# mckerrigan/shadow

Measured on AMD Instinct MI355X. Metric: source-paths/sec, higher is better.
Workload: dtype f64; 1 GPU; c4_as50k: Barabasi-Albert Internet-like topology, all-pairs latency/reliability table (BASELINE.json configs[3]); n_vertices=50000, n_edges=550000, n_edges_nonloop=500000, csr_arcs=1000000, targets=50000, table_bytes=40000000000, parallelism=one GPU

## Files before the change

### shadow_amd/csrc/sssp_delta.hpp

```cpp
#pragma once
#include "common.hpp"

namespace shd {

constexpr int KD_P = 8;
static_assert(KD_P == 8, "owner markers are read as one u64 per lane");
constexpr int KD_TAIL = 4;
constexpr int KD_W = 8;
constexpr int KD_IMP = 192;
constexpr uint32_t KD_NONE = 0xFFFFFFFFu;
constexpr uint32_t KD_SRC_MARK = 0xFFFFFFFEu;

#define KD_GLOBAL __attribute__((address_space(1)))

#ifndef KD_NSEEDS
#define KD_NSEEDS 3
#endif
constexpr int KD_SEEDS = KD_NSEEDS;
#ifndef KD_NTLOAD
#define KD_NTLOAD 1
#endif
#ifndef KD_JUMPS
#define KD_JUMPS 1
#endif
// ... 9 lines not shown
};
static_assert(sizeof(KDJob) == 64, "one 64-byte job record");
constexpr uint32_t KD_EVTAG = 0xFFFF0000u;
typedef unsigned short kd_us2 __attribute__((ext_vector_type(2)));
typedef double kd_d2 __attribute__((ext_vector_type(2)));
typedef unsigned kd_u4 __attribute__((ext_vector_type(4)));
typedef unsigned kd_u2 __attribute__((ext_vector_type(2)));

struct DevDelta {
    int* next;
    const KDJob* __restrict__ jobs;
    const uint16_t* __restrict__ drow;
    uint16_t* drow_out;
    uint32_t* prow;
    long long rstride;
    int evcap;
    int* done;
    int n, nw;
    int nlight;
    int nnz;
    int bound;
    int delta;
    int fused;
    int rc;
    const int* __restrict__ row;
    const uint32_t* __restrict__ orec;
    const uint16_t* __restrict__ oridx;
    const int* __restrict__ lrow;
    const uint2* __restrict__ lrec;
    const double* __restrict__ rtab;
    int nrtab;
    int rone;
    int walk;
    int packed;
    const double* __restrict__ vf;
    const double* __restrict__ self_w;
    const double* __restrict__ self_r;
    int has_vf;
    int dflags;
    int seed_drop;
    unsigned long long* dbg;
    unsigned long long* stats;
};

constexpr int KD_NACC = 40;
#ifdef SHD_STAMPS
#define KD_ACCP (sm->acc)
#define KD_OUT (!(dflags & 1))
#define KD_DFLAGS g.dflags
#define KD_STAMP(slot) do { if (tid == 0) sm->acc[slot] = __builtin_amdgcn_s_memtime(); } while (0)
#define KD_COUNT(slot, x) do { if (lane == 0 && (x)) atomicAdd(&sm->acc[slot], (unsigned long long)(x)); } while (0)
#define KD_MARK() do { if (tid == 0) kd_t = __builtin_amdgcn_s_memtime(); } while (0)
#define KD_ACC(slot) do { if (tid == 0) { const unsigned long long t_ = __builtin_amdgcn_s_memtime(); sm->acc[slot] += t_ - kd_t; kd_t = t_; } } while (0)
#define KD_FLUSH() do { lds_barrier(); if (g.dbg && i >= 0) for (int q_ = tid; q_ < KD_NACC; q_ += B) g.dbg[(size_t)i * KD_NACC + q_] = sm->acc[q_]; lds_barrier(); if (tid < KD_NACC) sm->acc[tid] = 0; lds_barrier(); } while (0)
#else
#define KD_ACCP nullptr
#define KD_OUT true
#define KD_DFLAGS 0
#define KD_STAMP(slot) do { } while (0)
#define KD_COUNT(slot, x) do { } while (0)
#define KD_MARK() do { } while (0)
#define KD_ACC(slot) do { } while (0)
#define KD_FLUSH() do { } while (0)
#endif

struct KDOut {
    const KD_GLOBAL int* tgt;
    KD_GLOBAL double* lat_out;
    KD_GLOBAL double* rel_out;
    KD_GLOBAL double* row_min;
    int* err;
    KD_GLOBAL double* relv;
    const KD_GLOBAL double* rtab;
    const KD_GLOBAL double* vf;
    long long ld;
    int n, nw, nt, tsorted;
    unsigned rmask;
    int rc, walk, nrtab, rone, has_vf, dflags;
};

struct KDSmall {
    unsigned gmin[2];
    int head, tail;
    int busy;
    int nexit;
    int rtail, rdone;
    int qtail[2];
    int qcur[2];
    unsigned long long rmin;
    int deep;
    int next;
    int nev;
    int evovf;
    int tsorted;
    int jflag[3];
    int wnext;
    int wnext2, novf;
    KDJob job;
    KDJob njob;
    int njb;
    int wpar;
    const KDJob* jobs;
    int* qnext;
    const uint16_t* drow;
    uint32_t* prow;
    long long rstride;
    int* done;
    uint32_t* wsl[2];
    int ns;
    KDOut out;
#ifdef SHD_STAMPS
    unsigned long long acc[KD_NACC];
#endif
};

template <int B>
struct KDLayout {
    size_t tmask, tpre, wmark, wkey, wimp, dist, pend, fix, wmin, work, ring, rrec, qv, qbeg, rix, rtabl, total;
    int qcap;
    __host__ __device__ static KDLayout make(int n, int rc, int rr) {
        KDLayout L;
        const size_t nw = (size_t)(n + 63) / 64;
        size_t o = a16(sizeof(KDSmall));
        L.tmask = o; o += a16(8 * nw);
        L.tpre = o;  o += a16(4 * nw);
        L.dist = o;  o += a16(sizeof(uint16_t) * (size_t)(n + 1));
        L.rix = o;
        L.wmark = o; o += (size_t)(B / 64) * 8 * KD_P;
        L.wkey = o;  o += (size_t)(B / 64) * 64 * 4;
        L.wimp = o;  o += (size_t)(B / 64) * KD_IMP * 4;
        L.pend = o;  o += a16(8 * nw);
        L.fix = o;   o += a16(8 * nw);
        L.wmin = o;  o += a16(4 * nw);
        L.work = o;
        const size_t wbytes = a16(2 * (size_t)rc) + 8 * (size_t)rr;
        L.ring = o;
        L.rrec = o + a16(2 * (size_t)rc);
        L.qcap = (int)((wbytes - 16) / 6) & ~7;
        L.qv = o;
        L.qbeg = o + a16(2 * (size_t)L.qcap);
        o += wbytes;
        L.total = o;
        L.rtabl = a16(L.rix + (size_t)n);
        return L;
    }
};
constexpr int KD_MAXD = 32;
#ifndef KD_SDIV
#define KD_SDIV 8
#endif
#ifndef KD_SMIN
#define KD_SMIN 16
#endif
#ifndef KD_WDYN
#define KD_WDYN 1
#endif
#ifndef KD_WCAP
#define KD_WCAP 2
#endif
#ifndef KD_SEEDSPIN
#define KD_SEEDSPIN 8
#endif
#ifndef KD_WQ_N
#define KD_WQ_N 2
#endif
constexpr int KD_WQ = KD_WQ_N;
constexpr int KD_ONE = 254;
constexpr int KD_NAN = 255;
constexpr int KD_RR = 512;
template <int B>
constexpr int kd_rr() { return B >= 1024 ? KD_RR : 256; }

__host__ __device__ inline size_t kd_ws_stride(int n) {
    return a16(sizeof(double) * n) + a16(sizeof(uint32_t) * (n + 8)) + a16(8 * (size_t)n) + 256 +
           a16(sizeof(uint32_t) * (n + 8));
}
__host__ __device__ inline size_t kd_ws_wpr1(int n) {
    return a16(sizeof(double) * n) + a16(sizeof(uint32_t) * (n + 8)) + a16(8 * (size_t)n) + 256;
}
__host__ __device__ inline long long kd_row_stride(int n) { return ((long long)n + 2 + 7) & ~7ll; }

__device__ inline void lds_barrier() { asm volatile("s_waitcnt lgkmcnt(0)\n\ts_barrier" ::: "memory"); }
__device__ inline void wait_stores() { asm volatile("s_waitcnt vmcnt(0)" ::: "memory"); }

__device__ inline unsigned kd_wave_min(unsigned x) {
#pragma unroll
    for (int d = 32; d >= 1; d >>= 1) x = min(x, (unsigned)__shfl_xor((int)x, d, 64));
    return x;
}

__device__ inline unsigned kd_wave_min_dpp(unsigned x) {
    int v = (int)x;
    const int inf = (int)0xFFFFFFFFu;
    v = (int)min((unsigned)v, (unsigned)__builtin_amdgcn_update_dpp(inf, v, 0x111, 0xF, 0xF, false));
    v = (int)min((unsigned)v, (unsigned)__builtin_amdgcn_update_dpp(inf, v, 0x112, 0xF, 0xF, false));
    v = (int)min((unsigned)v, (unsigned)__builtin_amdgcn_update_dpp(inf, v, 0x114, 0xF, 0xF, false));
    v = (int)min((unsigned)v, (unsigned)__builtin_amdgcn_update_dpp(inf, v, 0x118, 0xF, 0xF, false));
    v = (int)min((unsigned)v, (unsigned)__builtin_amdgcn_update_dpp(inf, v, 0x142, 0xA, 0xF, false));
    v = (int)min((unsigned)v, (unsigned)__builtin_amdgcn_update_dpp(inf, v, 0x143, 0xC, 0xF, false));
    return (unsigned)__builtin_amdgcn_readlane(v, 63);
}

__device__ inline int kd_wave_incl_sum(int x) {
    x += __builtin_amdgcn_update_dpp(0, x, 0x111, 0xF, 0xF, false);
    x += __builtin_amdgcn_update_dpp(0, x, 0x112, 0xF, 0xF, false);
    x += __builtin_amdgcn_update_dpp(0, x, 0x114, 0xF, 0xF, false);
    x += __builtin_amdgcn_update_dpp(0, x, 0x118, 0xF, 0xF, false);
    x += __builtin_amdgcn_update_dpp(0, x, 0x142, 0xA, 0xF, false);
    x += __builtin_amdgcn_update_dpp(0, x, 0x143, 0xC, 0xF, false);
    return x;
}

__device__ inline int kd_wave_incl_max(int x) {
    x = max(x, __builtin_amdgcn_update_dpp(0, x, 0x111, 0xF, 0xF, false));
    x = max(x, __builtin_amdgcn_update_dpp(0, x, 0x112, 0xF, 0xF, false));
// ... 57 lines not shown
        if (act) {
            uint32_t old = dist32[v >> 1];
            for (;;) {
                if (nd >= ((old >> sh) & 0xFFFFu)) break;
                const uint32_t got = atomicCAS(&dist32[v >> 1], old, (old & ~(0xFFFFu << sh)) | (nd << sh));
                if (got == old) { won = true; break; }
                old = got;
            }
        }
        const bool push = won && nd < T;
        if (won && nd >= T) { atomicOr(&pend[v >> 6], 1ull << (v & 63)); atomicMin(&wmin[v >> 6], nd); }
        const unsigned long long pm = __ballot(push);
        if (pm) {
            const int ctot = __popcll(pm);
            int qb = 0;
            if (lane == 0) qb = atomicAdd(tail, ctot);
            qb = __builtin_amdgcn_readfirstlane(qb);
            const int qk = max(0, min(ctot, rc - qb));
            const int rk = __popcll(pm & (upto >> 1));
            if (push && rk < qk) { ring[qb + rk] = (uint16_t)v; atomicAnd(&pend[v >> 6], ~(1ull << (v & 63))); }
            if (push && rk >= qk) { atomicOr(&pend[v >> 6], 1ull << (v & 63)); atomicMin(&wmin[v >> 6], nd); }
#ifdef SHD_STAMPS
            if (lane == 0 && ctot > qk) atomicAdd(&sm_acc[14], (unsigned long long)(ctot - qk));
#endif
        }
    }
    __builtin_amdgcn_wave_barrier();
}


#define SEED_VIEW()                                                                                   \
    const int nseed = __builtin_amdgcn_readfirstlane(sm->job.nseed);                                   \
    int su[KD_SEEDS], sslot[KD_SEEDS];                                                                 \
    unsigned wsu[KD_SEEDS], rsu[KD_SEEDS];                                                             \
    const uint16_t* sdrow[KD_SEEDS];                                                                   \
    const uint32_t* sprow[KD_SEEDS];                                                                   \
    _Pragma("unroll") for (int q_ = 0; q_ < KD_SEEDS; q_++) {                                          \
        const int sl_ = __builtin_amdgcn_readfirstlane(q_ < nseed ? sm->job.seed[q_] : 0);             \
        const unsigned wr_ = (unsigned)__builtin_amdgcn_readfirstlane(q_ < nseed ? sm->job.wr[q_] : 0); \
        su[q_] = __builtin_amdgcn_readfirstlane(q_ < nseed ? sm->job.u[q_] : -1);                      \
        sslot[q_] = sl_; wsu[q_] = wr_ & 0xFFFFu;                                                      \
        rsu[q_] = (unsigned)__builtin_amdgcn_readfirstlane(q_ < nseed ? sm->job.rec[q_] : 0);          \
        sdrow[q_] = g.drow + (size_t)sl_ * g.rstride;                                                  \
        sprow[q_] = g.prow + (size_t)sl_ * g.rstride;                                                  \
    }                                                                                                  \
    (void)sslot; (void)rsu; (void)sprow; (void)su

__device__ inline int kd_next_source(int* ctr, int* slot, int tid, bool all_queued = false) {
    if (tid == 0) *slot = (all_queued ? 0 : (int)gridDim.x) + atomicAdd(ctr, 1);
    __syncthreads();
    const int i = *slot;
    __syncthreads();
    return i;
}

template <int B>
__device__ __attribute__((noinline)) void kd_output(const int i, const int s, const double cs, const double sw_s,
                                                    const double sr_s, const KD_GLOBAL uint32_t* __restrict__ wpr) {
    extern __shared__ __attribute__((aligned(16))) char smem[];
    constexpr int RR = kd_rr<B>();
    KDSmall* sm = reinterpret_cast<KDSmall*>(smem);
    auto uni = [](auto x) __attribute__((always_inline)) {
        using T = decltype(x);
        if constexpr (sizeof(T) == 8) {
            unsigned long long b;
            __builtin_memcpy(&b, &x, 8);
            b = (unsigned long long)(unsigned)__builtin_amdgcn_readfirstlane((int)(unsigned)b) |
                ((unsigned long long)(unsigned)__builtin_amdgcn_readfirstlane((int)(unsigned)(b >> 32)) << 32);
            T y;
            __builtin_memcpy(&y, &b, 8);
            return y;
        } else {
            return (T)__builtin_amdgcn_readfirstlane((int)x);
        }
    };
    const KDOut& O = sm->out;
    const KD_GLOBAL int* __restrict__ const tgt = uni(O.tgt);
    KD_GLOBAL double* __restrict__ const lat_out = uni(O.lat_out);
    KD_GLOBAL double* __restrict__ const rel_out = uni(O.rel_out);
    KD_GLOBAL double* __restrict__ const row_min = uni(O.row_min);
    int* __restrict__ const err = uni(O.err);
    KD_GLOBAL double* __restrict__ const relv = uni(O.relv);
    const KD_GLOBAL double* __restrict__ const rtab = uni(O.rtab);
    const KD_GLOBAL double* __restrict__ const vf = uni(O.vf);
    const long long ld = uni(O.ld);
    const int n = uni(O.n), nw = uni(O.nw), nt = uni(O.nt), tsorted = uni(O.tsorted);
    const unsigned rmask = uni(O.rmask);
    const int rc = uni(O.rc), walk = uni(O.walk), nrtab = uni(O.nrtab), rone = uni(O.rone);
    const int has_vf = uni(O.has_vf), dflags = uni(O.dflags);
    const KDLayout<B> L = KDLayout<B>::make(n, rc, RR);
    const int tid = threadIdx.x, lane = tid & 63;
    uint16_t* dist = reinterpret_cast<uint16_t*>(smem + L.dist);
    unsigned long long* pend = reinterpret_cast<unsigned long long*>(smem + L.pend);
    unsigned long long* fix = reinterpret_cast<unsigned long long*>(smem + L.fix);
    uint16_t* qv = reinterpret_cast<uint16_t*>(smem + L.qv);
    const unsigned long long* tmask = reinterpret_cast<const unsigned long long*>(smem + L.tmask);
    const unsigned* tpre = reinterpret_cast<const unsigned*>(smem + L.tpre);
    const int qcap = L.qcap;
    auto tpos = [&](int v) __attribute__((always_inline)) {
        const unsigned long long wd = tmask[v >> 6], bit = 1ull << (v & 63);
        return (wd & bit) ? (int)tpre[v >> 6] + __popcll(wd & (bit - 1ull)) : -1;
    };
    struct { int walk; const KD_GLOBAL double* rtab; int nrtab; const KD_GLOBAL double* vf; int has_vf; } g = {walk, rtab, nrtab, vf, has_vf};
#ifdef SHD_STAMPS
    unsigned long long kd_t = __builtin_amdgcn_s_memtime();
#endif
    (void)lane; (void)dflags;
    KD_GLOBAL double* lrow = lat_out && i >= 0 ? lat_out + (long long)i * ld : nullptr;
    KD_GLOBAL double* rrow = rel_out && i >= 0 ? rel_out + (long long)i * ld : nullptr;
    double lmin = INFINITY;
    auto lat_of = [&](int t) __attribute__((always_inline)) {
        double Lv;
        if (t < 0 || t >= n) { raise_err(err, SHD_ROUTE_EINVAL); Lv = NAN; }
        else if (t == s) {
            if (isnan(sw_s)) { raise_err(err, SHD_ROUTE_ENOEDGE); Lv = NAN; }
            else { Lv = 0.0 + sw_s; lmin = fmin(lmin, Lv); }
        } else if (dist[t] == 0xFFFFu) { raise_err(err, SHD_ROUTE_EUNREACH); Lv = NAN; }
        else { Lv = (double)dist[t]; lmin = fmin(lmin, Lv); }
        return Lv;
    };
    const bool walks = g.walk && rrow;
    wait_stores();
    __syncthreads();
    if (tsorted) {
        const int lpar = (int)(((uintptr_t)lrow >> 3) & 1);
        const int wv = tid >> 6;
        for (int b0 = 256 * wv; b0 < (i >= 0 ? n : 0); b0 += 256 * (B / 64)) {
#pragma unroll
            for (int p = 0; p < 2; p++) {
                const int v = b0 + 128 * p + 2 * lane;
                if (v >= n) continue;
                const unsigned long long wd = tmask[v >> 6];
                const int sh = v & 63;
                const int j = (int)tpre[v >> 6] + __popcll(wd & ((1ull << sh) - 1ull));
                const uint32_t d2 = *reinterpret_cast<const uint32_t*>(dist + v);
                int jq[2];
                double Lq[2];
                int jn = j;
#pragma unroll
                for (int h = 0; h < 2; h++) {
                    const int vv = v + h;
                    const bool tg = vv < n && ((wd >> (sh + h)) & 1ull);
                    jq[h] = tg ? jn++ : -1;
                    const unsigned d = (d2 >> (16 * h)) & 0xFFFFu;
                    double Lv = 0.0;
                    if (tg) {
                        if (vv == s) {
                            if (isnan(sw_s)) { raise_err(err, SHD_ROUTE_ENOEDGE); Lv = NAN; }
                            else { Lv = 0.0 + sw_s; lmin = fmin(lmin, Lv); }
                        } else if (d == 0xFFFFu) { raise_err(err, SHD_ROUTE_EUNREACH); Lv = NAN; }
                        else { Lv = (double)d; lmin = fmin(lmin, Lv); }
                    }
                    Lq[h] = Lv;
                }
                if (!lrow || !KD_OUT) continue;
                const int ja = jq[0], jb = jq[1];
                if (ja >= 0 && jb == ja + 1 && !((ja + lpar) & 1))
                    __builtin_nontemporal_store(kd_d2{Lq[0], Lq[1]}, reinterpret_cast<KD_GLOBAL kd_d2*>(lrow + ja));
                else {
                    if (ja >= 0) __builtin_nontemporal_store(Lq[0], lrow + ja);
                    if (jb >= 0) __builtin_nontemporal_store(Lq[1], lrow + jb);
                }
            }
        }
    } else {
        for (int j = tid; j < (i >= 0 ? nt : 0); j += B) {
            const double Lv = lat_of(tgt[j]);
            if (lrow && KD_OUT) __builtin_nontemporal_store(Lv, lrow + j);
        }
    }
    const bool queued = sm->jobs != nullptr;
    if (tid == 0) {
        sm->deep = 0; sm->rmin = kInfBits; sm->wnext = 0; sm->wnext2 = 0; sm->novf = 0;
        if (queued) sm->njb = atomicAdd(sm->qnext, 1);
    }
    __syncthreads();
    const int njb = queued ? __builtin_amdgcn_readfirstlane(sm->njb) : -1;
    if (tid < 16 && njb >= 0) {
        const int x = njb < sm->ns ? ((const KD_GLOBAL int*)(sm->jobs + njb))[tid] : (tid == 3 ? 0 : -1);
        reinterpret_cast<int*>(&sm->njob)[tid] = x;
    }

    KD_ACC(18);
    uint16_t* parv = dist;
    if (walks) {
        uint8_t* rixl = reinterpret_cast<uint8_t*>(smem + L.rix);
        double* rtl = reinterpret_cast<double*>(smem + L.rtabl);
        for (int k = tid; k < 256; k += B)
            rtl[k] = k < g.nrtab ? g.rtab[k] : k == KD_ONE ? 1.0 : NAN;
        auto copy_trip = [&](const int v0, const auto& pr) __attribute__((always_inline)) {
            constexpr int NQ = sizeof(pr) / sizeof(pr[0]);
            uint2 dv[NQ];
#pragma unroll
            for (int q = 0; q < NQ; q++) dv[q] = *reinterpret_cast<const uint2*>(dist + min(v0 + q * 4 * B, (n - 1) & ~3));
#pragma unroll
            for (int q = 0; q < NQ; q++) {
                const int vb = v0 + q * 4 * B;
                if (vb >= n) continue;
                uint32_t pw[2] = {0u, 0u}, rw = 0u;
#pragma unroll
                for (int h = 0; h < 4; h++) {
                    const int v = vb + h;
                    const uint32_t p = h == 0 ? pr[q].x : h == 1 ? pr[q].y : h == 2 ? pr[q].z : pr[q].w;
                    const uint32_t d = ((h < 2 ? dv[q].x : dv[q].y) >> (16 * (h & 1))) & 0xFFFFu;
                    const bool src_v = v == s, unr = !src_v && d == 0xFFFFu;
                    const uint32_t pv = src_v || unr ? (uint32_t)s : (p & 0xFFFFu);
                    const uint32_t ri = min((p >> 16) & rmask, (uint32_t)(g.nrtab - 1));
                    const uint32_t rx = src_v ? (uint32_t)KD_ONE : unr ? (uint32_t)KD_NAN
                                        : ri == (uint32_t)rone ? (uint32_t)KD_ONE : ri;
                    pw[h >> 1] |= pv << (16 * (h & 1));
                    rw |= rx << (8 * h);
                }
                if (vb + 4 <= n) {
                    *reinterpret_cast<uint2*>(parv + vb) = make_uint2(pw[0], pw[1]);
                    *reinterpret_cast<uint32_t*>(rixl + vb) = rw;
                } else {
                    for (int h = 0; h < n - vb; h++) {
                        parv[vb + h] = (uint16_t)((pw[h >> 1] >> (16 * (h & 1))) & 0xFFFFu);
                        rixl[vb + h] = (uint8_t)((rw >> (8 * h)) & 0xFFu);
                    }
                }
            }
        };
        auto load_trip = [&](const int v0, auto& pr) __attribute__((always_inline)) {
            constexpr int NQ = sizeof(pr) / sizeof(pr[0]);
#pragma unroll
// ... 307 lines not shown
            double xp[4], xv[4];
#pragma unroll
            for (int q = 0; q < 4; q++) {
                xp[q] = relv[p4[q]];
                xv[q] = relv[v4[q] >= 0 ? v4[q] : 0];
            }
#pragma unroll
            for (int q = 0; q < 4; q++)
                if (v4[q] >= 0) relv[v4[q]] = xp[q] * (-xv[q]);
        }
        wait_stores();
        KD_ACC(14);
        lds_barrier();
        for (int k = tid; k < nw; k += B) {
            const unsigned long long r = fix[k];
            if (r) pend[k] &= ~r;
        }
        lds_barrier();
        KD_ACC(15);
    }
    KD_STAMP(3);

    if (rrow) {
        for (int j0 = tid; j0 < nt; j0 += B * 4) {
            int t4[4];
            double x4[4], f4[4];
#pragma unroll
            for (int q = 0; q < 4; q++) {
                const int j = j0 + q * B;
                t4[q] = j < nt ? tgt[j] : s;
            }
#pragma unroll
            for (int q = 0; q < 4; q++) {
                const int t = (t4[q] >= 0 && t4[q] < n) ? t4[q] : s;
                x4[q] = relv[t];
                f4[q] = g.has_vf ? g.vf[t] : (double)NAN;
            }
#pragma unroll
            for (int q = 0; q < 4; q++) {
                const int j = j0 + q * B;
                if (j >= nt) continue;
                const int t = t4[q];
                double Rv = NAN;
                if (t >= 0 && t < n) {
                    if (t == s) Rv = isnan(sw_s) ? NAN : cs * sr_s;
                    else Rv = isnan(f4[q]) ? x4[q] : x4[q] * f4[q];
                }
                if (KD_OUT) __builtin_nontemporal_store(Rv, rrow + j);
            }
        }
    }
    }
    if (row_min && i >= 0) {
#pragma unroll
        for (int d = 32; d >= 1; d >>= 1) lmin = fmin(lmin, __shfl_xor(lmin, d, 64));
        if (lane == 0 && lmin < INFINITY) atomicMin(&sm->rmin, as_u(lmin));
        __syncthreads();
        if (tid == 0) row_min[i] = as_d(sm->rmin);
    }
}

#define KD_KERNEL_PARAMS                                                                                   \
    DevDelta g, const int* __restrict__ src, int ns, const int* __restrict__ tgt, int nt, long long ld,     \
        double* __restrict__ lat_out, double* __restrict__ rel_out, double* __restrict__ row_min,          \
        int* __restrict__ err, char* __restrict__ ws, size_t ws_stride
template <int B>
__device__ __attribute__((always_inline)) inline void kd_rows_body(KD_KERNEL_PARAMS) {
    extern __shared__ __attribute__((aligned(16))) char smem[];
    const int n = g.n, nw = g.nw;
    constexpr int RR = kd_rr<B>();
    const KDLayout<B> L = KDLayout<B>::make(n, g.rc, RR);
    KDSmall* sm = reinterpret_cast<KDSmall*>(smem);
    const int tid = threadIdx.x, lane = tid & 63, wid = tid >> 6;
    uint32_t* wkey = reinterpret_cast<uint32_t*>(smem + L.wkey) + wid * 64;
    uint32_t* wimp = reinterpret_cast<uint32_t*>(smem + L.wimp) + wid * KD_IMP;
    uint16_t* dist = reinterpret_cast<uint16_t*>(smem + L.dist);
    uint32_t* wmark = reinterpret_cast<uint32_t*>(smem + L.wmark) + wid * 2 * KD_P;
    unsigned long long* pend = reinterpret_cast<unsigned long long*>(smem + L.pend);
    unsigned* wmin = reinterpret_cast<unsigned*>(smem + L.wmin);
    unsigned long long* fix = reinterpret_cast<unsigned long long*>(smem + L.fix);
    uint16_t* ring = reinterpret_cast<uint16_t*>(smem + L.ring);
    uint2* rrec = reinterpret_cast<uint2*>(smem + L.rrec);
    uint16_t* qv = reinterpret_cast<uint16_t*>(smem + L.qv);
    int* qbeg = reinterpret_cast<int*>(smem + L.qbeg);
    unsigned long long* tmask = reinterpret_cast<unsigned long long*>(smem + L.tmask);
    unsigned* tpre = reinterpret_cast<unsigned*>(smem + L.tpre);
    const unsigned delta = (unsigned)g.delta;
    const int qcap = L.qcap;
    const unsigned wmask = g.packed ? 0xFFu : 0xFFFFu;
    const unsigned rmask = g.packed ? 0xFFu : 0xFFFFu;
    const __amdgpu_buffer_rsrc_t orsrc =
        __builtin_amdgcn_make_buffer_rsrc(const_cast<uint32_t*>(g.orec), (short)0, g.nnz * 4, 0x00020000);
    const int rc = g.rc;
    constexpr int NW = B / 64;
    const bool writer = wid == NW - 1;
    double* relv = reinterpret_cast<double*>(ws + (size_t)blockIdx.x * ws_stride);
    uint32_t* const wslice = reinterpret_cast<uint32_t*>(ws + (size_t)blockIdx.x * ws_stride + a16(sizeof(double) * n));
    uint2* const evl = reinterpret_cast<uint2*>(ws + (size_t)blockIdx.x * ws_stride + a16(sizeof(double) * n) +
                                                a16(sizeof(uint32_t) * (n + 8)));
#ifdef SHD_STAMPS
    if (tid < KD_NACC) sm->acc[tid] = 0;
    __syncthreads();
#endif
    const unsigned long long upto = lane == 63 ? ~0ull : ((2ull << lane) - 1ull);

    for (int k = tid; k < nw; k += B) tmask[k] = 0ull;
    if (tid == 0) sm->tsorted = 1;
    __syncthreads();
    for (int j = tid; j < nt; j += B) {
        const int t = tgt[j];
        const bool ok = t >= 0 && t < n && (j == 0 || tgt[j - 1] < t);
        if (!ok) sm->tsorted = 0;
        else atomicOr(&tmask[t >> 6], 1ull << (t & 63));
    }
    __syncthreads();
    if (wid == 0) {
        int run = 0;
        for (int k0 = 0; k0 < nw; k0 += 64) {
            const int k = k0 + lane;
            const int c = k < nw ? __popcll(tmask[k]) : 0;
            const int incl = kd_wave_incl_sum(c);
            if (k < nw) tpre[k] = (unsigned)(run + incl - c);
            run += __builtin_amdgcn_readlane(incl, 63);
        }
    }
    __syncthreads();
    const bool tsorted = __builtin_amdgcn_readfirstlane(sm->tsorted) != 0;

    const bool queued = g.jobs != nullptr;
    if (tid == 0) {
        sm->njb = -1; sm->wpar = 0;
        sm->jobs = g.jobs; sm->qnext = g.next; sm->drow = g.drow; sm->prow = g.prow; sm->rstride = g.rstride;
        sm->done = g.done; sm->ns = ns;
        sm->wsl[0] = wslice;
        sm->wsl[1] = reinterpret_cast<uint32_t*>(ws + (size_t)blockIdx.x * ws_stride + kd_ws_wpr1(n));
        KDOut& o = sm->out;
        o.tgt = (const KD_GLOBAL int*)tgt; o.lat_out = (KD_GLOBAL double*)lat_out; o.rel_out = (KD_GLOBAL double*)rel_out;
        o.row_min = (KD_GLOBAL double*)row_min; o.err = err; o.relv = (KD_GLOBAL double*)relv;
        o.rtab = (const KD_GLOBAL double*)g.rtab; o.vf = (const KD_GLOBAL double*)g.vf; o.ld = ld;
        o.n = n; o.nw = nw; o.nt = nt; o.tsorted = tsorted ? 1 : 0; o.rmask = rmask; o.rc = g.rc; o.walk = g.walk;
        o.nrtab = g.nrtab; o.rone = g.rone; o.has_vf = g.has_vf; o.dflags = KD_DFLAGS;
    }
    for (int jb = queued ? kd_next_source(g.next, &sm->next, tid, true) : (int)blockIdx.x; jb < ns;
         jb = sm->njb >= 0 ? sm->njb : kd_next_source(g.next, &sm->next, tid, queued)) {
        if (tid < 16) {
            int x;
            if (sm->njb >= 0) x = reinterpret_cast<const int*>(&sm->njob)[tid];
            else if (g.jobs) x = reinterpret_cast<const int*>(g.jobs + jb)[tid];
            else x = tid == 0 ? jb : tid == 1 ? src[jb] : tid == 2 ? -1 : 0;
            reinterpret_cast<int*>(&sm->job)[tid] = x;
        }
        if (tid == 0) sm->wpar ^= 1;
        __syncthreads();
        if (tid == 0) sm->njb = -1;
        const int i = sm->job.row, s = sm->job.s;
        {
            bool bad = s < 0 || s >= n || sm->job.nseed < 0 || sm->job.nseed > KD_SEEDS;
            for (int q = 0; q < KD_SEEDS; q++)
                if (q < sm->job.nseed) bad = bad || sm->job.u[q] < 0 || sm->job.u[q] >= n || sm->job.seed[q] < 0;
            if (bad) {
                if (tid == 0) raise_err(err, SHD_ROUTE_EINVAL);
                __syncthreads();
                continue;
            }
        }
        auto wpr_of = [&]() __attribute__((always_inline)) {
            const int st = __builtin_amdgcn_readfirstlane(sm->job.store);
            return st >= 0 ? g.prow + (size_t)st * g.rstride : sm->wsl[__builtin_amdgcn_readfirstlane(sm->wpar)];
        };
        const double fs = g.vf[s];
        const double cs = isnan(fs) ? 1.0 : 1.0 * fs;
        const double sw_s = g.self_w[s], sr_s = g.self_r[s];
    kd_restart:
#ifdef SHD_STAMPS
        unsigned long long kd_t = 0;
#endif
        KD_MARK();
#ifdef SHD_STAMPS
        wait_stores();
        KD_ACC(9);
#endif
        const bool seeded = __builtin_amdgcn_readfirstlane(sm->job.nseed) > 0;
        if (seeded) {
            uint32_t* const wpr = wpr_of();
            if (tid == 0) {
#ifdef SHD_STAMPS
// ... 39 lines not shown
                for (int q = 0; q < KD_SEEDS; q++) {
                    if (q < nseed) {
                        if constexpr (B >= 1024 && KD_NTLOAD) {
                            typedef unsigned u2v __attribute__((ext_vector_type(2)));
                            const u2v d2 = __builtin_nontemporal_load(reinterpret_cast<const u2v*>(sdrow[q] + vl));
                            const kd_u4 p4 = __builtin_nontemporal_load(reinterpret_cast<const kd_u4*>(sprow[q] + vl));
                            dq[q] = make_uint2(d2.x, d2.y);
                            pq[q] = make_uint4(p4.x, p4.y, p4.z, p4.w);
                        } else {
                            dq[q] = *reinterpret_cast<const uint2*>(sdrow[q] + vl);
                            pq[q] = *reinterpret_cast<const uint4*>(sprow[q] + vl);
                        }
                    } else {
                        dq[q] = make_uint2(0xFFFFFFFFu, 0xFFFFFFFFu);
                        pq[q] = make_uint4(KD_NONE, KD_NONE, KD_NONE, KD_NONE);
                    }
                }
                uint32_t dw[2], rw[4];
#pragma unroll
                for (int h = 0; h < 4; h++) {
                    const int v = v0 + h;
                    unsigned dbest = 0xFFFFu, kbest = 0xFFFFFFFFu;
                    uint32_t rbest = KD_NONE;
#pragma unroll
                    for (int q = 0; q < KD_SEEDS; q++) {
                        const uint32_t d2 = (h < 2) ? dq[q].x : dq[q].y;
                        const unsigned d = (h & 1) ? (d2 >> 16) : (d2 & 0xFFFFu);
                        const unsigned c = q < nseed ? min(0xFFFFu, wsu[q] + d) : 0xFFFFFu;
                        const uint32_t p = kd_comp(pq[q], h);
                        const uint32_t r = v == su[q] ? rsu[q] : p;
                        const uint32_t k = __builtin_amdgcn_perm(~r, r, 0x07010002u);
                        if (c < dbest || (c == dbest && k < kbest)) { dbest = c; kbest = k; rbest = r; }
                    }
                    if (v >= n) dbest = 0xFFFFu;
                    if (v == s) rbest = KD_SRC_MARK;
                    if (h & 1) dw[h >> 1] |= dbest << 16;
                    else dw[h >> 1] = dbest;
                    rw[h] = rbest;
                }
                *reinterpret_cast<uint2*>(dist + v0) = make_uint2(dw[0], dw[1]);
                *reinterpret_cast<uint4*>(wpr + v0) = make_uint4(rw[0], rw[1], rw[2], rw[3]);
            }
            wait_stores();
        } else {
            for (int v = tid; v < (n + 2) / 2; v += B) reinterpret_cast<uint32_t*>(dist)[v] = 0xFFFFFFFFu;
        }
        for (int k = tid; k < nw; k += B) { pend[k] = 0ull; wmin[k] = 0xFFFFFFFFu; fix[k] = 0ull; }
        for (int q = tid; q < RR; q += B) rrec[q] = make_uint2(0u, 0xFFFFFFFFu);
        if (lane < 2 * KD_P) wmark[lane] = 0u;
        if (tid == 0) {
            sm->gmin[0] = sm->gmin[1] = 0xFFFFFFFFu;
            sm->rtail = sm->rdone = 0;
            sm->nev = 0; sm->evovf = 0;
            wpr_of()[s] = KD_SRC_MARK;
        }
        lds_barrier();
        KD_ACC(29);
        KD_STAMP(0);
        if (tid == 0) {
            dist[s] = 0;
            pend[s >> 6] = 1ull << (s & 63);
            wmin[s >> 6] = 0;
        }
        lds_barrier();

        unsigned T = delta;
        int par = 0;
        const int ncomp = NW - 1;
        int wnev = 0;
        KD_MARK();
        for (;;) {
            KD_COUNT(5, tid == 0 ? 1 : 0);
            {
                unsigned m0 = 0xFFFFFFFFu;
                for (int k = tid; k < nw; k += B) m0 = min(m0, wmin[k]);
                const unsigned wm = kd_wave_min_dpp(m0);
                if (lane == 0 && wm != 0xFFFFFFFFu) atomicMin(&sm->gmin[par], wm);
            }
            for (int q = tid; q < rc; q += B) ring[q] = 0xFFFFu;
            if (tid == 0) { sm->gmin[par ^ 1] = 0xFFFFFFFFu; sm->head = sm->tail = 0; sm->busy = 0; sm->nexit = 0; }
            lds_barrier();
            const unsigned m = sm->gmin[par];
            if (m == 0xFFFFFFFFu) break;
            if (m >= T) T = (m / delta + 1) * delta;
            KD_ACC(11);
            for (int k0 = 0; k0 < nw; k0 += B) {
                const int k = k0 + tid;
                unsigned long long bits = 0ull, take = 0ull;
                unsigned rest = 0xFFFFFFFFu;
                const bool act = k < nw && wmin[k] < T;
                if (act) {
                    bits = pend[k];
                    unsigned long long b = bits;
                    while (b) {
                        int v4[4];
                        pop4(&b, k, v4);
                        unsigned d4[4];
#pragma unroll
                        for (int q = 0; q < 4; q++) d4[q] = ld16(dist, v4[q] >= 0 ? v4[q] : n);
#pragma unroll
                        for (int q = 0; q < 4; q++) {
                            if (v4[q] < 0) continue;
                            if (d4[q] < T) take |= 1ull << (v4[q] & 63);
                            else rest = min(rest, d4[q]);
                        }
                    }
// ... 333 lines not shown
            SEED_VIEW();
            auto d0 = [&](int v) __attribute__((always_inline)) {
                unsigned x = 0xFFFFu;
#pragma unroll
                for (int q = 0; q < KD_SEEDS; q++)
                    if (q < nseed) x = min(x, min(0xFFFFu, wsu[q] + (unsigned)sdrow[q][v]));
                return x;
            };
            KD_ACC(27);
            uint32_t* key = reinterpret_cast<uint32_t*>(relv);
            auto event = [&](int e, int& v, uint32_t& ke) __attribute__((always_inline)) {
                const uint2 r = evl[e];
                v = (int)r.y;
                const int p = (int)(r.x & 0xFFFFu);
                const unsigned w = r.x >> 24, dv = ld16(dist, v);
                if (dv != d0(v) || ld16(dist, p) + w != dv) { v = -1; return; }
                ke = ((0xFFu - w) << 24) | ((uint32_t)p << 8) | ((r.x >> 16) & 0xFFu);
            };
            for (int e = tid; e < nev; e += B) {
                int v; uint32_t ke = 0;
                event(e, v, ke);
                if (v >= 0) {
                    const uint32_t b = wpr[v];
                    const unsigned pb = b & 0xFFFFu, wb = ld16(dist, v) - ld16(dist, (int)pb);
                    key[v] = ((0xFFu - wb) << 24) | (pb << 8) | ((b >> 16) & 0xFFu);
                }
            }
            wait_stores();
            lds_barrier();
            for (int e = tid; e < nev; e += B) {
                int v; uint32_t ke = 0;
                event(e, v, ke);
                if (v >= 0) atomicMin(&key[v], ke);
            }
            wait_stores();
            lds_barrier();
            for (int e = tid; e < nev; e += B) {
                int v; uint32_t ke = 0;
                event(e, v, ke);
                if (v >= 0) {
                    const uint32_t k = __hip_atomic_load(&key[v], __ATOMIC_RELAXED, __HIP_MEMORY_SCOPE_AGENT);
                    wpr[v] = ((k >> 8) & 0xFFFFu) | ((k & 0xFFu) << 16) | ((0xFFu - (k >> 24)) << 24);
                }
            }
            wait_stores();
            lds_barrier();
            KD_ACC(28);
        }
        KD_STAMP(1);
        KD_MARK();

        const int last_arc = g.nlight > 0 ? g.nlight - 1 : 0;
        uint32_t* const wpr = wpr_of();
        if (tid == 0) {
            fix[s >> 6] &= ~(1ull << (s & 63));
            sm->qtail[0] = sm->qtail[1] = 0;
            sm->qcur[0] = sm->qcur[1] = 0;
        }
        for (int rnd = 0;; rnd ^= 1) {
            if (tid == 0) { sm->qtail[rnd ^ 1] = 0; sm->qcur[rnd ^ 1] = 0; }
            lds_barrier();
            for (int k0 = 0; k0 < nw; k0 += B) {
                const int k = k0 + tid;
                unsigned long long bits = k < nw ? fix[k] : 0ull;
                const int cnt = __popcll(bits);
                int incl = kd_wave_incl_sum(cnt);
                int base = 0;
                if (lane == 63 && incl) base = atomicAdd(&sm->qtail[rnd], incl);
                base = __builtin_amdgcn_readlane(base, 63);
                int pos = base + incl - cnt;
                unsigned long long b = bits, listed = 0ull;
                while (b && pos < qcap) {
                    const int bi = __ffsll((long long)b) - 1;
                    b &= b - 1;
                    qv[pos++] = (uint16_t)((k << 6) + bi);
                    listed |= 1ull << bi;
                }
                if (listed) fix[k] = bits & ~listed;
            }
            lds_barrier();
            const int cnt = min(sm->qtail[rnd], qcap);
            if (cnt == 0) break;
            for (int j0 = 0; j0 < cnt; j0 += B * 4) {
                int v4[4], a4[4], r4[4];
#pragma unroll
                for (int q = 0; q < 4; q++) {
                    const int j = j0 + q * B + tid;
                    v4[q] = j < cnt ? (int)qv[j] : -1;
                }
#pragma unroll
                for (int q = 0; q < 4; q++) {
                    const int vv = v4[q] >= 0 ? v4[q] : 0;
                    a4[q] = g.lrow[vv];
                    r4[q] = g.lrow[vv + 1];
                }
                uint2 rc[4][KD_TAIL];
#pragma unroll
                for (int q = 0; q < 4; q++)
#pragma unroll
                    for (int e = 0; e < KD_TAIL; e++) rc[q][e] = g.lrec[min(a4[q] + e, last_arc)];
                unsigned dt[4][KD_TAIL], d4[4];
#pragma unroll
                for (int q = 0; q < 4; q++) {
                    d4[q] = ld16(dist, v4[q] >= 0 ? v4[q] : 0);
#pragma unroll
                    for (int e = 0; e < KD_TAIL; e++) dt[q][e] = ld16(dist, (int)(rc[q][e].x & 0xFFFFu));
// ... 8 lines not shown
                        if (a4[q] + e < r4[q] && dt[q][e] + (rc[q][e].x >> 16) == d4[q]) {
                            f = e;
                            rec = (rc[q][e].x & 0xFFFFu) | (rc[q][e].y << 16) | (g.packed ? (rc[q][e].x >> 16) << 24 : 0u);
                        }
                    out_a[q] = rec;
                    if (v4[q] >= 0 && f < 0) {
                        if (r4[q] - a4[q] > KD_TAIL) {
                            const int at = atomicAdd(&sm->qcur[rnd], 1);
                            qbeg[at] = v4[q];
                            v4[q] = -1;
                        } else raise_err(err, SHD_ROUTE_EUNREACH);
                    }
                }
#pragma unroll
                for (int q = 0; q < 4; q++)
                    if (v4[q] >= 0) wpr[v4[q]] = out_a[q];
            }
            lds_barrier();
            const int nlong = sm->qcur[rnd];
            for (int j = wid; j < nlong; j += B / 64) {
                const int v = qbeg[j];
                const unsigned dv = ld16(dist, v);
                const int r1 = g.lrow[v + 1];
                uint32_t fr = KD_NONE;
                for (int a0 = g.lrow[v] + KD_TAIL; a0 < r1 && fr == KD_NONE; a0 += 64) {
                    const int a = a0 + lane;
                    const uint2 rc = g.lrec[min(a, last_arc)];
                    const bool tight = a < r1 && ld16(dist, (int)(rc.x & 0xFFFFu)) + (rc.x >> 16) == dv;
                    const unsigned long long tm = __ballot(tight);
                    if (tm) fr = (uint32_t)__builtin_amdgcn_readlane((int)((rc.x & 0xFFFFu) | (rc.y << 16) | (g.packed ? (rc.x >> 16) << 24 : 0u)),
                                                                  __ffsll((long long)tm) - 1);
                }
                if (lane == 0) {
                    if (fr == KD_NONE) raise_err(err, SHD_ROUTE_EUNREACH);
                    wpr[v] = fr;
                }
            }
        }
        KD_ACC(16);
        KD_ACC(17);
        const int store = __builtin_amdgcn_readfirstlane(sm->job.store);
        if (store >= 0) {
            uint16_t* dr = g.drow_out + (size_t)store * g.rstride;
            for (int v0 = 8 * tid; v0 <= n; v0 += 8 * B)
                *reinterpret_cast<uint4*>(dr + v0) = *reinterpret_cast<const uint4*>(dist + v0);
            wait_stores();
            __syncthreads();
            if (tid == 0) {
                __builtin_amdgcn_fence(__ATOMIC_RELEASE, "agent");
                asm volatile("s_waitcnt vmcnt(0)" ::: "memory");
                __hip_atomic_store(&g.done[store], 1, __ATOMIC_RELAXED, __HIP_MEMORY_SCOPE_AGENT);
            }
        }
        KD_STAMP(2);
        kd_output<B>(i, s, cs, sw_s, sr_s, (const KD_GLOBAL uint32_t*)wpr);
        lds_barrier();
        KD_STAMP(4);
        KD_FLUSH();
    }
}

template <int B>
__global__ __launch_bounds__(B) __attribute__((amdgpu_waves_per_eu(4))) void sssp_delta_kernel(KD_KERNEL_PARAMS) {
    kd_rows_body<B>(g, src, ns, tgt, nt, ld, lat_out, rel_out, row_min, err, ws, ws_stride);
}
template <int B>
__global__ __launch_bounds__(B) __attribute__((amdgpu_waves_per_eu(4))) void kd_plan_rows_kernel(KD_KERNEL_PARAMS) {
    kd_rows_body<B>(g, src, ns, tgt, nt, ld, lat_out, rel_out, row_min, err, ws, ws_stride);
}

template <int B>
inline size_t kd_lds_bytes(int n, int rc) { return KDLayout<B>::make(n, rc, kd_rr<B>()).total; }

template <int B>
inline bool kd_walk_fits(int n, int rc, int nrtab) {
    const KDLayout<B> L = KDLayout<B>::make(n, rc, kd_rr<B>());
    return nrtab <= KD_ONE && L.rtabl + 8 * 256 <= L.total;
}

}
```

Before: 1.212 million source-paths/s.

## Split post-SSSP phase into per-wave fixup and concurrent latency-row/store waves

For block sizes of 1024 or more, the predecessor fixup after the SSSP sweep is now done per wave, with each wave handling a slice of the fix bitmap independently and no block-wide barriers between rounds. The remaining waves at the same time copy the distance row to global memory and write the latency output row, taking 256-target chunks from an LDS atomic counter. Fixup waves join the latency work once they finish. This is meant to overlap the fixup with output writing and cut barrier-heavy rounds, at the cost of per-wave LDS queue partitions with smaller capacity and more code paths that must stay consistent.

```diff
diff --git a/shadow_amd/csrc/sssp_delta.hpp b/shadow_amd/csrc/sssp_delta.hpp
--- a/shadow_amd/csrc/sssp_delta.hpp
+++ b/shadow_amd/csrc/sssp_delta.hpp
@@ -85,6 +85,9 @@
 #define KD_COUNT(slot, x) do { if (lane == 0 && (x)) atomicAdd(&sm->acc[slot], (unsigned long long)(x)); } while (0)
 #define KD_MARK() do { if (tid == 0) kd_t = __builtin_amdgcn_s_memtime(); } while (0)
 #define KD_ACC(slot) do { if (tid == 0) { const unsigned long long t_ = __builtin_amdgcn_s_memtime(); sm->acc[slot] += t_ - kd_t; kd_t = t_; } } while (0)
+#define KD_WDECL(on) const bool kd_st = lane == 0 && (on); unsigned long long kd_w = __builtin_amdgcn_s_memtime(); (void)kd_st; (void)kd_w
+#define KD_WMARK() do { kd_w = __builtin_amdgcn_s_memtime(); } while (0)
+#define KD_WACC(slot) do { if (kd_st) { const unsigned long long t_ = __builtin_amdgcn_s_memtime(); sm->acc[slot] += t_ - kd_w; kd_w = t_; } } while (0)
 #define KD_FLUSH() do { lds_barrier(); if (g.dbg && i >= 0) for (int q_ = tid; q_ < KD_NACC; q_ += B) g.dbg[(size_t)i * KD_NACC + q_] = sm->acc[q_]; lds_barrier(); if (tid < KD_NACC) sm->acc[tid] = 0; lds_barrier(); } while (0)
 #else
 #define KD_ACCP nullptr
@@ -95,6 +98,9 @@
 #define KD_MARK() do { } while (0)
 #define KD_ACC(slot) do { } while (0)
 #define KD_FLUSH() do { } while (0)
+#define KD_WDECL(on) do { } while (0)
+#define KD_WMARK() do { } while (0)
+#define KD_WACC(slot) do { } while (0)
 #endif
 
 struct KDOut {
@@ -142,10 +148,17 @@
     uint32_t* wsl[2];
     int ns;
     KDOut out;
+    const int* lrow;
+    const uint2* lrec;
+    int nlight, packed;
+    int latblk;
 #ifdef SHD_STAMPS
     unsigned long long acc[KD_NACC];
 #endif
 };
+#ifndef SHD_STAMPS
+static_assert(sizeof(KDSmall) == 512, "LDS layout: KDSmall is eight 64-byte lines");
+#endif
 
 template <int B>
 struct KDLayout {
@@ -194,6 +207,12 @@
 #ifndef KD_SEEDSPIN
 #define KD_SEEDSPIN 8
 #endif
+#ifndef KD_BWAVES
+#define KD_BWAVES 8
+#endif
+#ifndef KD_BHELP
+#define KD_BHELP 1
+#endif
 #ifndef KD_WQ_N
 #define KD_WQ_N 2
 #endif
@@ -357,6 +376,104 @@
     const int i = *slot;
     __syncthreads();
     return i;
+}
+
+template <class T>
+__device__ __attribute__((always_inline)) inline T kd_uni(T x) {
+    if constexpr (sizeof(T) == 8) {
+        unsigned long long b;
+        __builtin_memcpy(&b, &x, 8);
+        b = (unsigned long long)(unsigned)__builtin_amdgcn_readfirstlane((int)(unsigned)b) |
+            ((unsigned long long)(unsigned)__builtin_amdgcn_readfirstlane((int)(unsigned)(b >> 32)) << 32);
+        T y;
+        __builtin_memcpy(&y, &b, 8);
+        return y;
+    } else {
+        return (T)__builtin_amdgcn_readfirstlane((int)x);
+    }
+}
+
+template <int B>
+__device__ __attribute__((noinline)) void kd_lat_row(const int i, const int s, const double sw_s) {
+    extern __shared__ __attribute__((aligned(16))) char smem[];
+    constexpr int RR = kd_rr<B>();
+    KDSmall* sm = reinterpret_cast<KDSmall*>(smem);
+    const KDOut& O = sm->out;
+    const KD_GLOBAL int* __restrict__ const tgt = kd_uni(O.tgt);
+    KD_GLOBAL double* __restrict__ const lat_out = kd_uni(O.lat_out);
+    int* __restrict__ const err = kd_uni(O.err);
+    const long long ld = kd_uni(O.ld);
+    const int n = kd_uni(O.n), nt = kd_uni(O.nt), tsorted = kd_uni(O.tsorted), dflags = kd_uni(O.dflags);
+    const KDLayout<B> L = KDLayout<B>::make(n, kd_uni(O.rc), RR);
+    const int lane = (int)threadIdx.x & 63;
+    auto next_block = [&]() __attribute__((always_inline)) {
+        int blk = 0;
+        if (lane == 0) blk = atomicAdd(&sm->latblk, 1);
+        return 256 * __builtin_amdgcn_readfirstlane(blk);
+    };
+    const uint16_t* dist = reinterpret_cast<const uint16_t*>(smem + L.dist);
+    const unsigned long long* tmask = reinterpret_cast<const unsigned long long*>(smem + L.tmask);
+    const unsigned* tpre = reinterpret_cast<const unsigned*>(smem + L.tpre);
+    (void)dflags;
+    KD_GLOBAL double* lrow = lat_out ? lat_out + (long long)i * ld : nullptr;
+    double lmin = INFINITY;
+    if (tsorted) {
+        const int lpar = (int)(((uintptr_t)lrow >> 3) & 1);
+        for (int b0 = next_block(); b0 < n; b0 = next_block()) {
+#pragma unroll
+            for (int p = 0; p < 2; p++) {
+                const int v = b0 + 128 * p + 2 * lane;
+                if (v >= n) continue;
+                const unsigned long long wd = tmask[v >> 6];
+                const int sh = v & 63;
+                const int j = (int)tpre[v >> 6] + __popcll(wd & ((1ull << sh) - 1ull));
+                const uint32_t d2 = *reinterpret_cast<const uint32_t*>(dist + v);
+                int jq[2];
+                double Lq[2];
+                int jn = j;
+#pragma unroll
+                for (int h = 0; h < 2; h++) {
+                    const int vv = v + h;
+                    const bool tg = vv < n && ((wd >> (sh + h)) & 1ull);
+                    jq[h] = tg ? jn++ : -1;
+                    const unsigned d = (d2 >> (16 * h)) & 0xFFFFu;
+                    double Lv = 0.0;
+                    if (tg) {
+                        if (vv == s) {
+                            if (isnan(sw_s)) { raise_err(err, SHD_ROUTE_ENOEDGE); Lv = NAN; }
+                            else { Lv = 0.0 + sw_s; lmin = fmin(lmin, Lv); }
+                        } else if (d == 0xFFFFu) { raise_err(err, SHD_ROUTE_EUNREACH); Lv = NAN; }
+                        else { Lv = (double)d; lmin = fmin(lmin, Lv); }
+                    }
+                    Lq[h] = Lv;
+                }
+                if (!lrow || !KD_OUT) continue;
+                const int ja = jq[0], jb = jq[1];
+                if (ja >= 0 && jb == ja + 1 && !((ja + lpar) & 1))
+                    __builtin_nontemporal_store(kd_d2{Lq[0], Lq[1]}, reinterpret_cast<KD_GLOBAL kd_d2*>(lrow + ja));
+                else {
+                    if (ja >= 0) __builtin_nontemporal_store(Lq[0], lrow + ja);
+                    if (jb >= 0) __builtin_nontemporal_store(Lq[1], lrow + jb);
+                }
+            }
+        }
+    } else {
+        for (int b0 = next_block(); b0 < nt; b0 = next_block())
+        for (int j = b0 + lane; j < min(nt, b0 + 256); j += 64) {
+            const int t = tgt[j];
+            double Lv;
+            if (t < 0 || t >= n) { raise_err(err, SHD_ROUTE_EINVAL); Lv = NAN; }
+            else if (t == s) {
+                if (isnan(sw_s)) { raise_err(err, SHD_ROUTE_ENOEDGE); Lv = NAN; }
+                else { Lv = 0.0 + sw_s; lmin = fmin(lmin, Lv); }
+            } else if (dist[t] == 0xFFFFu) { raise_err(err, SHD_ROUTE_EUNREACH); Lv = NAN; }
+            else { Lv = (double)dist[t]; lmin = fmin(lmin, Lv); }
+            if (lrow && KD_OUT) __builtin_nontemporal_store(Lv, lrow + j);
+        }
+    }
+#pragma unroll
+    for (int d = 32; d >= 1; d >>= 1) lmin = fmin(lmin, __shfl_xor(lmin, d, 64));
+    if (lane == 0 && lmin < INFINITY) atomicMin(&sm->rmin, as_u(lmin));
 }
 
 template <int B>
@@ -425,6 +542,7 @@
         return Lv;
     };
     const bool walks = g.walk && rrow;
+    if constexpr (B < 1024) {
     wait_stores();
     __syncthreads();
     if (tsorted) {
@@ -474,9 +592,12 @@
             if (lrow && KD_OUT) __builtin_nontemporal_store(Lv, lrow + j);
         }
     }
+    }
+    (void)lrow; (void)lat_of; (void)tsorted; (void)nt; (void)tgt;
     const bool queued = sm->jobs != nullptr;
     if (tid == 0) {
-        sm->deep = 0; sm->rmin = kInfBits; sm->wnext = 0; sm->wnext2 = 0; sm->novf = 0;
+        sm->deep = 0; sm->wnext = 0; sm->wnext2 = 0; sm->novf = 0;
+        if constexpr (B < 1024) sm->rmin = kInfBits;
         if (queued) sm->njb = atomicAdd(sm->qnext, 1);
     }
     __syncthreads();
@@ -890,15 +1011,158 @@
     }
     }
     if (row_min && i >= 0) {
-#pragma unroll
-        for (int d = 32; d >= 1; d >>= 1) lmin = fmin(lmin, __shfl_xor(lmin, d, 64));
-        if (lane == 0 && lmin < INFINITY) atomicMin(&sm->rmin, as_u(lmin));
+        if constexpr (B < 1024) {
+#pragma unroll
+            for (int d = 32; d >= 1; d >>= 1) lmin = fmin(lmin, __shfl_xor(lmin, d, 64));
+            if (lane == 0 && lmin < INFINITY) atomicMin(&sm->rmin, as_u(lmin));
+        }
         __syncthreads();
         if (tid == 0) row_min[i] = as_d(sm->rmin);
     }
 }
 
-#define KD_KERNEL_PARAMS                                                                                   \
+template <int B>
+__device__ __attribute__((noinline)) void kd_fixup(const int s_, KD_GLOBAL uint32_t* wpr_) {
+    const int s = kd_uni(s_);
+    KD_GLOBAL uint32_t* __restrict__ const wpr = kd_uni(wpr_);
+    extern __shared__ __attribute__((aligned(16))) char smem[];
+    constexpr int RR = kd_rr<B>();
+    KDSmall* sm = reinterpret_cast<KDSmall*>(smem);
+    const int n = kd_uni(sm->out.n), nw = kd_uni(sm->out.nw);
+    const KDLayout<B> L = KDLayout<B>::make(n, kd_uni(sm->out.rc), RR);
+    const int tid = threadIdx.x, lane = tid & 63, wid = tid >> 6;
+    const uint16_t* dist = reinterpret_cast<const uint16_t*>(smem + L.dist);
+    KD_WDECL(wid == 0);
+    {
+        unsigned long long* fix = reinterpret_cast<unsigned long long*>(smem + L.fix);
+        const int nlight = kd_uni(sm->nlight);
+        const __amdgpu_buffer_rsrc_t lrs =
+            __builtin_amdgcn_make_buffer_rsrc(const_cast<int*>(kd_uni(sm->lrow)), (short)0, (n + 1) * 4, 0x00020000);
+        const __amdgpu_buffer_rsrc_t ars =
+            __builtin_amdgcn_make_buffer_rsrc(const_cast<uint2*>(kd_uni(sm->lrec)), (short)0, nlight * 8, 0x00020000);
+        int* __restrict__ const err = kd_uni(sm->out.err);
+        const bool packed = kd_uni(sm->packed) != 0;
+        const int qw = L.qcap / KD_BWAVES;
+        uint16_t* const myq = reinterpret_cast<uint16_t*>(smem + L.qv) + wid * qw;
+        int* const myl = reinterpret_cast<int*>(smem + L.qbeg) + wid * qw;
+        const int lcap = qw / 2;
+        const int sword = s >> 6;
+        const unsigned long long sbit = 1ull << (s & 63);
+        for (;;) {
+            int cnt = 0;
+            for (int k0 = 64 * wid; k0 < nw && cnt < lcap; k0 += 64 * KD_BWAVES) {
+                const int k = k0 + lane;
+                const unsigned long long had = k < nw ? fix[k] : 0ull;
+                const unsigned long long bits = k == sword ? had & ~sbit : had;
+                const int c = __popcll(bits);
+                const int incl = kd_wave_incl_sum(c);
+                int pos = cnt + incl - c;
+                unsigned long long b = bits, listed = 0ull;
+                while (b && pos < lcap) {
+                    const int bi = __ffsll((long long)b) - 1;
+                    b &= b - 1;
+                    myq[pos++] = (uint16_t)((k << 6) + bi);
+                    listed |= 1ull << bi;
+                }
+                if ((bits & ~listed) != had) fix[k] = bits & ~listed;
+                cnt = min(lcap, cnt + __builtin_amdgcn_readlane(incl, 63));
+            }
+            if (cnt == 0) break;
+            __builtin_amdgcn_wave_barrier();
+            int nlong = 0;
+            for (int j0 = 0; j0 < cnt; j0 += 64 * 4) {
+                int v4[4], a4[4], r4[4];
+#pragma unroll
+                for (int q = 0; q < 4; q++) {
+                    const int j = j0 + q * 64 + lane;
+                    v4[q] = j < cnt ? (int)myq[j] : -1;
+                }
+#pragma unroll
+                for (int q = 0; q < 4; q++) {
+                    const int vv = v4[q] >= 0 ? v4[q] : 0;
+                    const kd_u2 lr = __builtin_amdgcn_raw_buffer_load_b64(lrs, (uint32_t)vv << 2, 0, 0);
+                    a4[q] = (int)lr.x;
+                    r4[q] = (int)lr.y;
+                }
+                kd_u2 rc[4][KD_TAIL];
+#pragma unroll
+                for (int q = 0; q < 4; q++)
+#pragma unroll
+                    for (int e = 0; e < KD_TAIL; e++) rc[q][e] = __builtin_amdgcn_raw_buffer_load_b64(ars, (uint32_t)a4[q] << 3, 8 * e, 0);
+                unsigned dt[4][KD_TAIL], d4[4];
+#pragma unroll
+                for (int q = 0; q < 4; q++) {
+                    d4[q] = ld16(dist, v4[q] >= 0 ? v4[q] : 0);
+#pragma unroll
+                    for (int e = 0; e < KD_TAIL; e++) dt[q][e] = ld16(dist, (int)(rc[q][e].x & 0xFFFFu));
+                }
+#pragma unroll
+                for (int q = 0; q < 4; q++) {
+                    int f = -1;
+                    uint32_t rec = KD_NONE;
+#pragma unroll
+                    for (int e = KD_TAIL - 1; e >= 0; e--)
+                        if (a4[q] + e < r4[q] && dt[q][e] + (rc[q][e].x >> 16) == d4[q]) {
+                            f = e;
+                            rec = (rc[q][e].x & 0xFFFFu) | (rc[q][e].y << 16) | (packed ? (rc[q][e].x >> 16) << 24 : 0u);
+                        }
+                    const bool miss = v4[q] >= 0 && f < 0;
+                    const bool lng = miss && r4[q] - a4[q] > KD_TAIL;
+                    if (miss && !lng) raise_err(err, SHD_ROUTE_EUNREACH);
+                    const unsigned long long lm = __ballot(lng);
+                    if (lng) {
+                        const int at = nlong + (int)__builtin_amdgcn_mbcnt_hi((unsigned)(lm >> 32), __builtin_amdgcn_mbcnt_lo((unsigned)lm, 0u));
+                        myl[2 * at] = a4[q] + KD_TAIL;
+                        myl[2 * at + 1] = (int)((unsigned)v4[q] | ((unsigned)(r4[q] - a4[q] - KD_TAIL) << 16));
+                    } else if (v4[q] >= 0) {
+                        wpr[v4[q]] = rec;
+                    }
+                    nlong += __popcll(lm);
+                }
+            }
+            KD_WACC(16);
+            __builtin_amdgcn_wave_barrier();
+            const int gi = lane >> 3, sub = lane & 7;
+            for (int j0 = 0; j0 < nlong; j0 += 8) {
+                const bool have = j0 + gi < nlong;
+                const int e0 = have ? myl[2 * (j0 + gi)] : 0;
+                const unsigned e1 = have ? (unsigned)myl[2 * (j0 + gi) + 1] : 0u;
+                const int v = (int)(e1 & 0xFFFFu);
+                int a0 = e0;
+                const int r1 = e0 + (int)(e1 >> 16);
+                const unsigned dv = ld16(dist, v);
+                uint32_t fr = KD_NONE;
+                bool open = have && a0 < r1;
+                while (__ballot(open)) {
+                    const int a = a0 + sub;
+                    const kd_u2 ra = __builtin_amdgcn_raw_buffer_load_b64(ars, (uint32_t)a << 3, 0, 0);
+                    const kd_u2 rb = __builtin_amdgcn_raw_buffer_load_b64(ars, (uint32_t)a << 3, 64, 0);
+                    const unsigned da = ld16(dist, (int)(ra.x & 0xFFFFu)), db = ld16(dist, (int)(rb.x & 0xFFFFu));
+                    const bool ta = open && a < r1 && da + (ra.x >> 16) == dv;
+                    const bool tb = open && a + 8 < r1 && db + (rb.x >> 16) == dv;
+                    const unsigned ma = (unsigned)(__ballot(ta) >> (8 * gi)) & 0xFFu;
+                    const unsigned mb = (unsigned)(__ballot(tb) >> (8 * gi)) & 0xFFu;
+                    const uint32_t ca = (ra.x & 0xFFFFu) | (ra.y << 16) | (packed ? (ra.x >> 16) << 24 : 0u);
+                    const uint32_t cb = (rb.x & 0xFFFFu) | (rb.y << 16) | (packed ? (rb.x >> 16) << 24 : 0u);
+                    const unsigned mm = ma ? ma : mb;
+                    const int from = 8 * gi + (mm ? __ffs((int)mm) - 1 : 0);
+                    const uint32_t got = (uint32_t)__shfl((int)(ma ? ca : cb), from, 64);
+                    if (open && mm) { fr = got; open = false; }
+                    if (open) { a0 += 16; open = a0 < r1; }
+                }
+                if (sub == 0 && have) {
+                    if (fr == KD_NONE) raise_err(err, SHD_ROUTE_EUNREACH);
+                    wpr[v] = fr;
+                }
+            }
+            KD_WACC(17);
+        }
+        wait_stores();
+        KD_WACC(16);
+    }
+}
+
+#define KD_KERNEL_PARAMS                                                                              \
     DevDelta g, const int* __restrict__ src, int ns, const int* __restrict__ tgt, int nt, long long ld,     \
         double* __restrict__ lat_out, double* __restrict__ rel_out, double* __restrict__ row_min,          \
         int* __restrict__ err, char* __restrict__ ws, size_t ws_stride
@@ -970,6 +1234,10 @@
         sm->njb = -1; sm->wpar = 0;
         sm->jobs = g.jobs; sm->qnext = g.next; sm->drow = g.drow; sm->prow = g.prow; sm->rstride = g.rstride;
         sm->done = g.done; sm->ns = ns;
+        if constexpr (B >= 1024) {
+            sm->lrow = g.lrow; sm->lrec = g.lrec;
+            sm->nlight = g.nlight; sm->packed = g.packed;
+        }
         sm->wsl[0] = wslice;
         sm->wsl[1] = reinterpret_cast<uint32_t*>(ws + (size_t)blockIdx.x * ws_stride + kd_ws_wpr1(n));
         KDOut& o = sm->out;
@@ -1115,6 +1383,10 @@
             sm->gmin[0] = sm->gmin[1] = 0xFFFFFFFFu;
             sm->rtail = sm->rdone = 0;
             sm->nev = 0; sm->evovf = 0;
+            if constexpr (B >= 1024) {
+                sm->rmin = kInfBits;
+                sm->latblk = 0;
+            }
             wpr_of()[s] = KD_SRC_MARK;
         }
         lds_barrier();
@@ -1554,6 +1826,34 @@
 
         const int last_arc = g.nlight > 0 ? g.nlight - 1 : 0;
         uint32_t* const wpr = wpr_of();
+        if constexpr (B >= 1024) {
+        static_assert(KD_BWAVES >= 1 && KD_BWAVES < NW, "B waves and store waves");
+        constexpr int NSW = NW - KD_BWAVES;
+        const int store = __builtin_amdgcn_readfirstlane(sm->job.store);
+        KD_WDECL(wid == 0 || wid == KD_BWAVES);
+        if (wid < KD_BWAVES) {
+            kd_fixup<B>(s, (KD_GLOBAL uint32_t*)wpr);
+            KD_WMARK();
+            if (KD_BHELP && wid > 0 && i >= 0) kd_lat_row<B>(i, s, sw_s);
+        } else {
+            if (store >= 0) {
+                uint16_t* dr = g.drow_out + (size_t)store * g.rstride;
+                for (int v0 = 8 * (tid - 64 * KD_BWAVES); v0 <= n; v0 += 8 * 64 * NSW)
+                    *reinterpret_cast<uint4*>(dr + v0) = *reinterpret_cast<const uint4*>(dist + v0);
+                wait_stores();
+            }
+            KD_WACC(37);
+            if (i >= 0) kd_lat_row<B>(i, s, sw_s);
+            KD_WACC(38);
+        }
+        lds_barrier();
+        if (wid == 0) KD_WACC(39);
+        if (store >= 0 && tid == 0) {
+            __builtin_amdgcn_fence(__ATOMIC_RELEASE, "agent");
+            asm volatile("s_waitcnt vmcnt(0)" ::: "memory");
+            __hip_atomic_store(&g.done[store], 1, __ATOMIC_RELAXED, __HIP_MEMORY_SCOPE_AGENT);
+        }
+        } else {
         if (tid == 0) {
             fix[s >> 6] &= ~(1ull << (s & 63));
             sm->qtail[0] = sm->qtail[1] = 0;
@@ -1668,6 +1968,7 @@
                 __hip_atomic_store(&g.done[store], 1, __ATOMIC_RELAXED, __HIP_MEMORY_SCOPE_AGENT);
             }
         }
+        }
         KD_STAMP(2);
         kd_output<B>(i, s, cs, sw_s, sr_s, (const KD_GLOBAL uint32_t*)wpr);
         lds_barrier();
```

After: 1.243 million source-paths/s, median of 6. +2.6%, better.
